# modichirag/GSM-VI

Hardware: AMD Instinct MI355X
Metric: GSM updates/sec at D=1024,B=32 (dense-cov gsm_update, fp64) (higher is better)
Workload: dtype f64; 1 GPU; BASELINE configs[2]: D=1024 dense-cov Gaussian target, B=32, one GSM update per step; D=1024, B=32, instances=21, ring_bytes=352321536, launch=hipGraph(90 x 21 updates/replay + 1 x 7), warmup_steps_run=28, parallelism=single GPU

## Files before the change

### gsm-vi_amd/csrc/gsmvi_abi.hip

```cpp
#include <hip/hip_runtime.h>

#include <cstdio>
#include <cstdlib>
#include <cstring>
#include <string>

#include "../../include/gsmvi_hip.h"
#include "../../include/gsmvi_hip_debug.h"

void gsmvi_launch_panel_partial(hipStream_t st, hipEvent_t* ev, int MT, dim3 grid, int D, int ncols, int nrows,
                                const double* A, int lda, const double* shift, double alpha, const double* M,
                                int ldm, double* Pp, int chunks_per_wg, int a_vec_ok);
void gsmvi_launch_panel_finish(hipStream_t st, hipEvent_t* ev, int D, int nrows, int KC, const double* Pp,
                               const double* addvec, double* Out, int ldo, int ncols_out);
void gsmvi_launch_gsm_scalars(hipStream_t st, hipEvent_t* ev, int D, int B, int KC, const double* X, int ldx,
                              const double* G, int ldg, const double* mu0, const double* Pp, double* rec,
                              int ldrec);
size_t gsmvi_cov_update_lds_bytes(int SB);
hipError_t gsmvi_cov_update_prepare();
hipError_t gsmvi_bam_prepare();
hipError_t gsmvi_batched_prepare();
hipError_t gsmvi_bam_batched_prepare();
hipError_t gsmvi_psis_batched_prepare();
hipError_t gsmvi_psis_loo_batched_prepare();
hipError_t gsmvi_psis_loo_softmax_batched_prepare();
hipError_t gsmvi_softmax_predict_batched_prepare();
void gsmvi_launch_gsm_cov_update(hipStream_t st, hipEvent_t* ev, int D, int B, const double* rec, int ldrec,
                                 const double* mu0, const double* S0, int lds0, double* S, int lds, double* mu_out,
                                 int SB, int s_vec_ok, int row0, int nrows);
int gsmvi_panel_t_product(struct gsmvi_ctx* ctx, hipStream_t st, int D, int B, const double* A, int lda,
                          const double* M, int ldm, int mrows, double* Pp, int* kc_out);
void gsmvi_launch_commit(hipStream_t st, int D, const int* info, const double* mu_new, const double* S_new,
                         int lds_new, double* mu, double* S, int lds, int* n_reverts);
void gsmvi_launch_panel_fast(hipStream_t st, hipEvent_t* ev, int MT, dim3 grid, int D, int nrows, const double* A,
                             int lda, const double* shift, double alpha, const double* M, int ldm, double* Pp,
                             int chunks_per_wg, int ncols, unsigned long long* stamps, double* Out, int ldo,
                             const double* addvec, const struct gsmvi_panel_extras* px);
bool gsmvi_launch_gsm_scalars_fast(hipStream_t st, hipEvent_t* ev, int D, int B, int KC, const double* X, int ldx,
                                   const double* G, int ldg, const double* mu0, const double* Pp, double* rec,
                                   int ldrec, int nt, unsigned long long* stamps);
bool gsmvi_launch_gsm_cov_sym(hipStream_t st, hipEvent_t* ev, int D, int B, const double* rec, int ldrec,
                              const double* mu0, const double* S0, int lds0, double* S, int lds, double* mu_out,
                              int dbg, unsigned long long* stamps, int num_cu);
void gsmvi_launch_panel_fast_part(hipStream_t st, hipEvent_t* ev, dim3 grid, int D, int B, const double* G, int ldg,
                                  const double* S0, int lds0, double* Pp, int chunks_per_wg, const double* X, int ldx,
                                  const double* mu0, double* Qg, double* Qm, int chw, bool qm_whole, int stream,
                                  unsigned long long* stamps);
void gsmvi_launch_gsm_cov_sym_slabs(hipStream_t st, hipEvent_t* ev, int D, int B, const struct gsm_slab_src& fs, const double* mu0,
                                    const double* S0, int lds0, double* S, int lds, double* mu_out, int kct, bool fold,
                                    bool s0_last, bool store_wt, bool qm_whole, unsigned long long* stamps);
int gsmvi_cov_sym_pairs(int nt);
int gsmvi_panel_fast_chunk(int MT);
int gsmvi_potrf_impl(struct gsmvi_ctx* ctx, hipStream_t st, int D, const double* S, int lds, double* R, int ldr,
                     int* info_dev);
int gsmvi_gram_impl(hipStream_t st, int D, const double* F, int ldf, double* C, int ldc, double shift, const double* shift_dev);
int gsmvi_whiten_impl(hipStream_t st, int D, int nrows, const double* R, int ldr, const double* X, int ldx,
                      const double* mu, double* Z, int ldz, double* logdiag);
int gsmvi_factor_impl(struct gsmvi_ctx* ctx, hipStream_t st, int D, int B, const double* Z, int ldz, const double* X,
                      int ldx, const double* G, int ldg, const double* mu0, const double* F0, int ldf0, double* mu,
                      double* F, int ldf, int* info_dev, int* n_reverts_dev);
int gsmvi_factor_local_impl(struct gsmvi_ctx* ctx, hipStream_t st, int D, int Bl, const double* Z, int ldz,
                            const double* X, int ldx, const double* G, int ldg, const double* mu0, const double* F0,
                            int ldf0, double* rec, int ldrec);
int gsmvi_factor_apply_impl(struct gsmvi_ctx* ctx, hipStream_t st, int D, int B, const double* Z, int ldz,
                            const double* rec, int ldrec, const double* mu0, const double* F0, int ldf0, double* mu,
                            double* F, int ldf, int* info_dev, int* n_reverts_dev);
int gsmvi_factor_apply_cols_impl(struct gsmvi_ctx* ctx, hipStream_t st, int D, int B, int col0, int ncols, const double* Z,
                                 int ldz, const double* W, int ldw, const double* X, int ldx, const double* mu0,
                                 const double* F0c, int ldf0, double* mu, double* Fc, int ldf, int* info_dev,
                                 int* n_reverts_dev);
int gsmvi_bam_impl(struct gsmvi_ctx* ctx, hipStream_t st, int D, int B, const double* X, int ldx,
                   const double* G, int ldg, const double* mu0, const double* S0, int lds0, double reg,
                   double jitter, double* mu, double* S, int lds, int* info_dev);
int gsmvi_bam_factor_impl(gsmvi_ctx* ctx, hipStream_t st, int D, int B, const double* Z, int ldz, const double* X, int ldx,
                          const double* G, int ldg, const double* mu0, const double* F0, int ldf0, double reg, double* mu,
                          double* F, int ldf, int* info_dev, int* n_reverts_dev);
int gsmvi_bam_factor_wq_partial_impl(gsmvi_ctx* ctx, hipStream_t st, int D, int B, int col0, int ncols, const double* G, int ldg,
                                     const double* F0c, int ldf0, double reg, double* Wq_part);
int gsmvi_bam_factor_apply_cols_impl(gsmvi_ctx* ctx, hipStream_t st, int D, int B, int col0, int ncols, const double* Z, int ldz,
                                     const double* X, int ldx, const double* G, int ldg, const double* Wq, const double* mu0,
                                     const double* F0c, int ldf0, double reg, double* mu, double* Fc, int ldf, int* info_dev,
                                     int* n_reverts_dev);

#include "gsmvi_ctx.h"
#include "gsmvi_panel_split.h"

static thread_local std::string g_last_error;

void gsmvi_set_error(const char* fmt, const char* a, const char* b) {
    char buf[512];
    snprintf(buf, sizeof buf, fmt, a ? a : "", b ? b : "");
    g_last_error = buf;
}

#define HIP_TRY(expr)                                                     \
    do {                                                                  \
        hipError_t e_ = (expr);                                           \
        if (e_ != hipSuccess) {                                           \
            gsmvi_set_error("%s failed: %s", #expr, hipGetErrorString(e_)); \
            return GSMVI_ERR_HIP;                                         \
        }                                                                 \
    } while (0)

// ... 156 lines not shown

int gsmvi_destroy(gsmvi_ctx* ctx) {
    if (!ctx) return GSMVI_OK;
    int prev_device = 0;
    (void)hipGetDevice(&prev_device);
    struct device_guard {
        int prev;
        ~device_guard() { (void)hipSetDevice(prev); }
    } guard{prev_device};
    (void)hipSetDevice(ctx->device);
    for (int k = 0; k < 8; ++k)
        if (ctx->ev[k]) (void)hipEventDestroy(ctx->ev[k]);
    if (ctx->ev_fork) (void)hipEventDestroy(ctx->ev_fork);
    if (ctx->ev_join) (void)hipEventDestroy(ctx->ev_join);
    if (ctx->side) (void)hipStreamDestroy(ctx->side);
    if (ctx->bam_hint_host) (void)hipHostFree(ctx->bam_hint_host);
    if (ctx->stamps) (void)hipFree(ctx->stamps);
    hipError_t e = hipFree(ctx->ws);
    delete ctx;
    if (e != hipSuccess) {
        gsmvi_set_error("hipFree failed: %s%s", hipGetErrorString(e), "");
        return GSMVI_ERR_HIP;
    }
    return GSMVI_OK;
}

int gsmvi_set_tuning(gsmvi_ctx* ctx, const char* name, int value) {
    BAD_ARG(!ctx || !name, "NULL argument");
    if (!strcmp(name, "panel_kc")) ctx->tune_panel_kc = value;
    else if (!strcmp(name, "update_sb")) ctx->tune_update_sb = value;
    else if (!strcmp(name, "no_fast")) ctx->tune_no_fast = value;
    else if (!strcmp(name, "direct_out")) ctx->tune_direct_out = value;
    else if (!strcmp(name, "rider")) ctx->tune_rider = value;
    else if (!strcmp(name, "potrf_split_m")) ctx->tune_potrf_split_m = value;
    else if (!strcmp(name, "potrf_dag")) ctx->tune_potrf_dag = value;
    else if (!strcmp(name, "panel_w4_min_D")) ctx->tune_panel_w4_min_D = value;
    else if (!strcmp(name, "potrf_spin")) ctx->tune_potrf_spin = value;
    else if (!strcmp(name, "potrf_workers")) ctx->tune_potrf_workers = value;
    else if (!strcmp(name, "wide")) ctx->tune_wide = value;
    else if (!strcmp(name, "wide_kc")) ctx->tune_wide_kc = value;
    else if (!strcmp(name, "fork_min_D")) ctx->tune_fork_min_D = value;
    else if (!strcmp(name, "gram_mt")) ctx->tune_gram_mt = value > 0 ? value : 4;
    else if (!strcmp(name, "bam_full")) ctx->tune_bam_full = value;
    else if (!strcmp(name, "bam_kenq")) ctx->tune_bam_kenq = value;
    else if (!strcmp(name, "bam_hint_slack")) ctx->tune_bam_hint_slack = value;
    else if (!strcmp(name, "rider_direct_max_D")) ctx->tune_rider_direct_max_D = value;
    else if (!strcmp(name, "chain_pair")) ctx->tune_chain_pair = value;
    else if (!strcmp(name, "bam_batched_pad")) ctx->tune_bam_batched_pad = value;
    else if (!strcmp(name, "lowrank_kp")) ctx->tune_lowrank_kp = value;
    else if (!strcmp(name, "bam_basis")) ctx->tune_bam_basis = value;
    else if (!strcmp(name, "scalars_nt")) ctx->tune_scalars_nt = value;
    else if (!strcmp(name, "gsm_two_launch")) ctx->tune_gsm_two_launch = value;
    else if (!strcmp(name, "cov_fold_diag")) ctx->tune_cov_fold_diag = value;
    else if (!strcmp(name, "cov_s0_last")) ctx->tune_cov_s0_last = value;
    else if (!strcmp(name, "cov_store_wt")) ctx->tune_cov_store_wt = value;
    else if (!strcmp(name, "panel_qm_whole")) ctx->tune_panel_qm_whole = value;
    else if (!strcmp(name, "panel_stream")) ctx->tune_panel_stream = value;
    else if (!strcmp(name, "cov_dbg")) ctx->tune_cov_dbg = value;
    else if (!strcmp(name, "timeline")) {
        if (value && !ctx->stamps) {
            HIP_TRY(hipMalloc(reinterpret_cast<void**>(&ctx->stamps), GSMVI_STAMP_WORDS * sizeof(unsigned long long)));
            HIP_TRY(hipMemset(ctx->stamps, 0, GSMVI_STAMP_WORDS * sizeof(unsigned long long)));
        }
        ctx->tune_timeline = value;
    }
    else {
        gsmvi_set_error("%s: unknown tuning knob %s", __func__, name);
        return GSMVI_ERR_BAD_ARG;
    }
    return GSMVI_OK;
}

int gsmvi_debug_stream_copy_f64(void* stream, double* dst, const double* src, size_t n) {
    BAD_ARG(!dst || !src || n < 2 || (n & 1) || (reinterpret_cast<uintptr_t>(dst) & 15u) || (reinterpret_cast<uintptr_t>(src) & 15u),
            "bad argument (16-byte aligned pointers, even n)");
    hipLaunchKernelGGL(k_stream_copy, dim3(2048), dim3(256), 0, static_cast<hipStream_t>(stream),
                       reinterpret_cast<const v2d_abi*>(src), reinterpret_cast<v2d_abi*>(dst), n / 2);
    return hipGetLastError() == hipSuccess ? GSMVI_OK : GSMVI_ERR_HIP;
}

int gsmvi_debug_read_stamps(gsmvi_ctx* ctx, unsigned long long* out, int n) {
    BAD_ARG(!ctx || !out || n < 1, "bad argument");
    HIP_TRY(hipDeviceSynchronize());
    if (ctx->tune_timeline && ctx->stamps) {
        BAD_ARG(n > GSMVI_STAMP_WORDS, "more words than the timeline buffer holds");
        HIP_TRY(hipMemcpy(out, ctx->stamps, sizeof(unsigned long long) * (size_t)n, hipMemcpyDeviceToHost));
        return GSMVI_OK;
    }
    HIP_TRY(hipMemcpy(out, ctx->pp, sizeof(unsigned long long) * (size_t)n, hipMemcpyDeviceToHost));
    return GSMVI_OK;
}

static double* ws_region(const gsmvi_ctx* ctx, int region) { return region == 0 ? ctx->pp : (region == 1 ? ctx->sg : ctx->small); }

int gsmvi_debug_read_workspace(gsmvi_ctx* ctx, int region, size_t offset, double* out, size_t n) {
    BAD_ARG(!ctx || !out || region < 0 || region > 2, "bad argument");
    const double* base = ws_region(ctx, region);
    HIP_TRY(hipDeviceSynchronize());
    HIP_TRY(hipMemcpy(out, base + offset, sizeof(double) * n, hipMemcpyDeviceToHost));
    return GSMVI_OK;
}

int gsmvi_debug_workspace_ptr(gsmvi_ctx* ctx, int region, double** out) {
    BAD_ARG(!ctx || !out || region < 0 || region > 2, "bad argument");
    *out = ws_region(ctx, region);
    return GSMVI_OK;
// ... 224 lines not shown
    return check_launch("k_gsm_scalars");
}

static bool gsm_two_launch_gate(const gsmvi_ctx* ctx, int D, int B, const double* X, int ldx, const double* G, int ldg,
                                const double* mu0, const double* S0, int lds0, const double* S, int lds, int* cpw_out,
                                int* kc_out, int* chw_out) {
    if (!ctx->tune_gsm_two_launch || ctx->tune_no_fast || ctx->tune_cov_dbg) return false;
    if (B != 16 && B != 32) return false;
    if (D % 256 != 0 || D > 1024) return false;
    if (ldx % 2 != 0 || ldg % 2 != 0 || lds0 % 2 != 0 || lds % 2 != 0) return false;
    if (!aligned16(X) || !aligned16(G) || !aligned16(mu0) || !aligned16(S0) || !aligned16(S)) return false;
    const int strips = D / 16, nchunks = D / 256;
    const gsmvi_panel_split sp = gsmvi_panel_split_k(strips, nchunks, ctx->tune_panel_kc, ctx->num_cu, GSMVI_MAX_KC);
    if (sp.kc > 4 || sp.kc * sp.cpw != nchunks) return false;
    *cpw_out = sp.cpw;
    *kc_out = sp.kc;
    *chw_out = 256;
    if (nchunks == 4 && ctx->tune_panel_kc <= 0) {
        *cpw_out = 1;
        *kc_out = 2;
        *chw_out = 512;
    }
    return true;
}

static int gsm_two_launch(gsmvi_ctx* ctx, hipStream_t hs, int D, int B, int cpw, int kc, int chw, const double* X, int ldx,
                          const double* G, int ldg, const double* mu0, const double* S0, int lds0, double* mu, double* S,
                          int lds) {
    const int strips = D / 16;
    double* Qg = ctx->sg;
    double* Qm = Qg + (size_t)B * kc * strips;
    ctx->px = gsmvi_panel_extras();
    ctx->px_used = 1;
    hipEvent_t* ev0 = ctx->stage_events(0);
    ctx->ev_valid[1] = 0;
    const bool qm_whole = chw == 512 && D == 1024 && ctx->tune_panel_qm_whole != 0;
    const int stream = (chw == 512 && D == 1024 && cpw == 1 && !qm_whole && ctx->tune_panel_stream != 0) ? (ctx->tune_panel_stream == 4 ? 4 : 2) : 0;
    gsmvi_launch_panel_fast_part(hs, ev0, dim3(strips, kc, chw == 512 ? B / 16 : 1), D, B, G, ldg, S0, lds0, ctx->pp, cpw, X, ldx, mu0, Qg, Qm, chw,
                                 qm_whole, stream, ctx->timeline_stamps(0));
    ctx->path |= GSMVI_PATH_PANEL_FAST | (chw == 512 ? GSMVI_PATH_PANEL_CHUNK512 : 0u) | (qm_whole ? GSMVI_PATH_PANEL_QM_WHOLE : 0u);
    int st = check_launch("k_panel_fast(partials)");
    if (st != GSMVI_OK) return st;
    gsm_slab_src fs;
    fs.X = X;
    fs.ldx = ldx;
    fs.Pp = ctx->pp;
    fs.Qg = Qg;
    fs.Qm = Qm;
    fs.KC = kc;
    fs.strips = strips;
    const bool fold = ctx->tune_cov_fold_diag >= 2 || (ctx->tune_cov_fold_diag == 1 && gsmvi_cov_sym_pairs(D / 32) >= ctx->num_cu);
    const bool s0_last = chw == 512 && ctx->tune_cov_s0_last != 0;
    const bool store_wt = chw == 512 && ctx->tune_cov_store_wt != 0 && (size_t)D * (size_t)lds * sizeof(double) < ((size_t)1 << 31);
    gsmvi_launch_gsm_cov_sym_slabs(hs, ctx->stage_events(2), D, B, fs, mu0, S0, lds0, S, lds, mu, chw == 512 ? 2 : 4, fold,
                                   s0_last, store_wt, qm_whole, ctx->timeline_stamps(2));
    ctx->path |= GSMVI_PATH_COV_SYM | GSMVI_PATH_GSM_TWO_LAUNCH | (fold ? GSMVI_PATH_COV_FOLD_DIAG : 0u) |
                 (s0_last ? GSMVI_PATH_COV_S0_LAST : 0u) | (store_wt ? GSMVI_PATH_COV_STORE_WT : 0u);
    return check_launch("k_gsm_cov_sym(slabs)");
}

int gsmvi_gsm_update_f64(gsmvi_ctx* ctx, void* stream, int D, int B, const double* X, int ldx, const double* G,
                         int ldg, const double* mu0, const double* S0, int lds0, double* mu, double* S, int lds) {
    int st = check_common(ctx, D, B, __func__);
    if (st != GSMVI_OK) return st;
    BAD_ARG(!X || !G || !mu0 || !S0 || !mu || !S, "NULL array");
    BAD_ARG(ldx < D || ldg < D || lds0 < D || lds < D, "leading dimension smaller than D");
    BAD_ARG(S == S0 || mu == mu0, "outputs must not alias inputs");
    hipStream_t hs = reinterpret_cast<hipStream_t>(stream);
    const int ldrec = 3 * D + (D & 1);
    int cpw2 = 0, kc2 = 0, chw2 = 0;
    if (gsm_two_launch_gate(ctx, D, B, X, ldx, G, ldg, mu0, S0, lds0, S, lds, &cpw2, &kc2, &chw2))
        return gsm_two_launch(ctx, hs, D, B, cpw2, kc2, chw2, X, ldx, G, ldg, mu0, S0, lds0, mu, S, lds);
    st = gsm_local_stage(ctx, hs, D, B, X, ldx, G, ldg, mu0, S0, lds0, ctx->sg, ldrec);
    if (st != GSMVI_OK) return st;
    return gsm_apply(ctx, hs, D, B, ctx->sg, ldrec, mu0, S0, lds0, mu, S, lds);
}

int gsmvi_gsm_record_len(int D) { return 3 * D + (D & 1); }

int gsmvi_gsm_update_general_f64(gsmvi_ctx* ctx, void* stream, int D, int B, const double* X, int ldx, const double* G,
                                 int ldg, const double* mu0, const double* S0, int lds0, double* mu, double* S, int lds) {
    int st = check_common(ctx, D, B, __func__);
    if (st != GSMVI_OK) return st;
    BAD_ARG(!X || !G || !mu0 || !S0 || !mu || !S, "NULL array");
    BAD_ARG(ldx < D || ldg < D || lds0 < D || lds < D, "leading dimension smaller than D");
    BAD_ARG(S == S0 || mu == mu0, "outputs must not alias inputs");
    hipStream_t hs = reinterpret_cast<hipStream_t>(stream);
    const int ldrec = 3 * D + (D & 1);
    int kc = 1;
    st = gsmvi_panel_t_product(ctx, hs, D, B, G, ldg, S0, lds0, D, ctx->pp, &kc);
    if (st != GSMVI_OK) return st;
    st = gsm_records(ctx, hs, D, B, kc, X, ldx, G, ldg, mu0, ctx->pp, ctx->sg, ldrec);
    if (st != GSMVI_OK) return st;
    const int SB = cov_update_sb(B, 0);
    const int s_vec_ok = (lds0 % 2 == 0) && (lds % 2 == 0) && aligned16(S0) && aligned16(S);
    ctx->path |= GSMVI_PATH_COV_GENERIC;
    gsmvi_launch_gsm_cov_update(hs, nullptr, D, B, ctx->sg, ldrec, mu0, S0, lds0, S, lds, mu, SB, s_vec_ok, 0, D);
    return check_launch("k_gsm_cov_update(general)");
}

int gsmvi_gsm_local_stage_f64(gsmvi_ctx* ctx, void* stream, int D, int B_local, const double* X, int ldx,
                              const double* G, int ldg, const double* mu0, const double* S0, int lds0, double* rec,
                              int ldrec) {
    int st = check_common(ctx, D, B_local, __func__);
    if (st != GSMVI_OK) return st;
    BAD_ARG(!X || !G || !mu0 || !S0 || !rec, "NULL array");
    BAD_ARG(ldx < D || ldg < D || lds0 < D || ldrec < 3 * D, "leading dimension too small");
    hipStream_t hs = reinterpret_cast<hipStream_t>(stream);
    return gsm_local_stage(ctx, hs, D, B_local, X, ldx, G, ldg, mu0, S0, lds0, rec, ldrec);
// ... 257 lines not shown
```

### gsm-vi_amd/csrc/gsmvi_ctx.h

```cpp
#pragma once
#include <hip/hip_runtime.h>
#include <cstddef>

#define GSMVI_MAX_KC 8
#define GSMVI_FACTOR_NMAX 256
#define GSMVI_STAMP_WORDS (4 * 4096)

struct gsmvi_panel_extras {
    const double* msl = nullptr;
    int kcm = 0;
    size_t mstride = 0;
    int ldsl = 0, msplit = 0;
    double* mfin = nullptr;
    int ldfin = 0;
    const double* sj_src = nullptr;
    int sj_kc = 0;
    size_t sj_stride = 0;
    int sj_len = 0;
    double* sj_dst = nullptr;
    int rd_on = 0, rd_n = 0, rd_B = 0, rd_kcg = 0, rd_jmode = 0;
    const double* rd_Gp = nullptr;
    double *rd_Kmat = nullptr, *rd_coef = nullptr;
    int* rd_bad = nullptr;
    unsigned long long* rd_stamps = nullptr;
// ... 14 lines not shown

struct bam_reg {
    double v;
    const double* p;
#if defined(__HIPCC__)
    __device__ __forceinline__ double get() const { return p ? *p : v; }
#endif
};

struct gsmf_bam_mean {
    const double* xbar;
    const double* sg_r1;
    bam_reg reg;
};

struct gsmvi_ctx {
    gsmvi_panel_extras px;
    int px_used = 0;
    unsigned path = 0;
    int tune_panel_w4_min_D = 2048;
    int colwin_0 = 0, colwin_n = 0;
    const double* potrf_w = nullptr;
    const double* potrf_r = nullptr;
    int potrf_w_n = 0;
    int tune_potrf_dag = 1;
    int tune_potrf_workers = 0;
    int tune_potrf_spin = 0;
    int tune_potrf_split_m = 0;
    int tune_wide = 1;
    int tune_wide_kc = 0;
    int tune_gram_mt = 1;
    int tune_rider = 1;
    int device = 0;
    int max_D = 0, max_B = 0;
    int num_cu = 256;
    int rmax = 0;
    void* ws = nullptr;
    size_t ws_bytes = 0;
    double* pp = nullptr;
    double* sg = nullptr;
    double *fo_Rt = nullptr, *fo_Tm = nullptr, *fo_Fs = nullptr;
    double* small = nullptr;
    int* ints = nullptr;
    double* gram_slabs = nullptr;
    int tune_panel_kc = 0;
    int tune_update_sb = 0;
    int tune_cov_dbg = 0;
    int tune_timeline = 0;
    unsigned long long* stamps = nullptr;
    int tune_direct_out = 1;
    int tune_scalars_nt = 0;
    int tune_no_fast = 0;
    int tune_cov_fold_diag = 1;
    int tune_cov_s0_last = 1;
    int tune_cov_store_wt = 1;
    int tune_panel_qm_whole = 0;
    int tune_panel_stream = 1;
    int tune_gsm_two_launch = 1;
    int* bam_hint_host = nullptr;
    int tune_bam_kenq = 0;
    int tune_bam_hint_slack = 1;
    int tune_rider_direct_max_D = 2048;
    int tune_bam_full = 0;
    int tune_lowrank_kp = 0;
    int tune_bam_batched_pad = 1;
    int tune_chain_pair = 1;
    gsmf_bam_mean bam_mean = {nullptr, nullptr, {0.0, nullptr}};
    int bam_mean_done = 0;
    const double* chain_r11 = nullptr;
    const double* chain_w11 = nullptr;
    const double* reg_dev = nullptr;
    int tune_bam_basis = 1;
    double* basis = nullptr;
    const double* chain_pi = nullptr;
    double* chain_x = nullptr;
    double* early = nullptr;
    int early_ready = 0;
    int profiling = 0;
    hipStream_t side = nullptr;
    hipEvent_t ev_fork = nullptr, ev_join = nullptr;
    int tune_fork_min_D = 3072;
    hipEvent_t ev[8] = {};
    int ev_valid[4] = {};

    unsigned long long* timeline_stamps(int kernel) {
        return (tune_timeline && stamps) ? stamps + (size_t)kernel * 4096 : nullptr;
    }

    hipEvent_t* stage_events(int stage) {
        if (!profiling) return nullptr;
        ev_valid[stage] = 1;
        return &ev[2 * stage];
    }
};

void gsmvi_panel_wide_split(int D, int tiles, int num_cu, int kc_force, int* kc_out, int* kper_out);
void gsmvi_launch_panel_wide(hipStream_t st, hipEvent_t* ev, bool transposed, int D, int nrows, const double* A, int lda,
                             const double* shift, double alpha, const double* M, int ldm, double* Pp, int kper, int kc,
                             int ncols);
int gsmvi_panel_product_nc(gsmvi_ctx* ctx, hipStream_t st, hipEvent_t* ev, int D, int ncols, int nrows,
                           const double* A, int lda, const double* shift, double alpha, const double* M, int ldm,
                           double* Pp, int* kc_out);
int gsmvi_panel_product_out(gsmvi_ctx* ctx, hipStream_t st, int D, int ncols, int nrows, const double* A, int lda,
                            const double* shift, double alpha, const double* M, int ldm, const double* addvec, double* Out,
                            int ldo);
int gsmvi_panel_finish(hipStream_t st, int ncols, int nrows, int kc, const double* Pp, const double* addvec,
// ... 16 lines not shown
```

### gsm-vi_amd/csrc/gsmvi_fast.hip

```cpp
#include "gsmvi_common.h"
#include "gsmvi_ctx.h"
#include "gsmvi_small16.h"
#include <hip/hip_ext.h>

#define GSMVI_LAUNCH(kern, grid, block, shmem, st, ev, ...)                                         \
    do {                                                                                           \
        if (ev)                                                                                    \
            hipExtLaunchKernelGGL(kern, grid, block, shmem, st, (ev)[0], (ev)[1], 0, __VA_ARGS__); \
        else                                                                                       \
            hipLaunchKernelGGL(kern, grid, block, shmem, st, __VA_ARGS__);                         \
    } while (0)

template <int NS>
__device__ __forceinline__ void panel_stream_chunk(double* As, int D, int nrows, const double* __restrict__ A, int lda, double alpha,
                                                   const double* __restrict__ M, int ldm, const gsmvi_panel_extras& px,
                                                   unsigned long long* __restrict__ stamps, v4d& acc, double& pq_g, double& pq_x,
                                                   double& pq_m) {
    static_assert(NS == 2 || NS == 4, "stages of the streamed left operand");
    constexpr int LDG = 514;
    constexpr int UPR = 32 / NS;
    constexpr int RPI = 64 / UPR;
    constexpr int IPS = 16 / RPI;
    constexpr int SPS = 16 / NS;
    const int tid = threadIdx.x, w = tid >> 6, l = tid & 63, c = l & 15, ks = l >> 4;
// ... 420 lines not shown
        gv[e] = G[(size_t)b * ldg + ic];
        mv0[e] = mu0[ic];
    }
    double p0 = 0.0, p1 = 0.0, sg[EPT], dd[EPT];
#pragma unroll
    for (int e = 0; e < EPT; ++e) {
        const int i = tid + NT * e;
        double t = 0.0;
#pragma unroll
        for (int kc = 0; kc < KCT; ++kc) t += (kc < KC) ? pp[e][kc] : 0.0;
        sg[e] = t;
        dd[e] = mv0[e] - xv[e];
        if (i < D) {
            p0 += gv[e] * t;
            p1 += dd[e] * gv[e];
        }
    }
    if (stamps && threadIdx.x == 0) stamps[(size_t)blockIdx.x * 8 + 1] = __builtin_amdgcn_s_memrealtime();
    p0 = wave_sum(p0);
    p1 = wave_sum(p1);
    const int w = tid >> 6;
    if ((tid & 63) == 0) {
        lds[2 * w] = p0;
        lds[2 * w + 1] = p1;
    }
    __syncthreads();
    double gSg = 0.0, mv = 0.0;
#pragma unroll
    for (int k = 0; k < NW; ++k) {
        gSg += lds[2 * k];
        mv += lds[2 * k + 1];
    }
    const double rho = 0.5 * sqrt(1.0 + 4.0 * (gSg + mv * mv)) - 0.5;
    const double den = 1.0 + rho + mv;
    const double beta = 1.0 / (1.0 + rho), c = (gSg - mv) / den;
    double* rb = rec + (size_t)b * ldrec;
#pragma unroll
    for (int e = 0; e < EPT; ++e) {
        const int i = tid + NT * e;
        if (i < D) {
            const double dmu = beta * ((sg[e] - dd[e]) - c * dd[e]);
            rb[i] = dd[e];
            rb[D + i] = dd[e] + dmu;
            rb[2 * D + i] = dmu;
        }
    }
    if (stamps) {
        asm volatile("s_waitcnt vmcnt(0)" ::: "memory");
        if (threadIdx.x == 0) stamps[(size_t)blockIdx.x * 8 + 3] = __builtin_amdgcn_s_memrealtime();
    }
}

typedef unsigned int v4u __attribute__((ext_vector_type(4)));
template <int SB, bool RAG, bool FROM_SLABS = false, int KCT = 4, bool FOLD = false, bool S0L = false, bool WT = false, bool QMW = false>
__global__ __launch_bounds__(512) __attribute__((amdgpu_waves_per_eu(FROM_SLABS ? 4 : 2))) void k_gsm_cov_sym(int D, int B, double invB, const double* __restrict__ rec, int ldrec,
                                                     const double* __restrict__ mu0,
                                                     const double* __restrict__ S0, int lds0,
                                                     double* __restrict__ S, int lds,
                                                     double* __restrict__ mu_out, int dbg,
                                                     unsigned long long* __restrict__ stamps, gsm_slab_src fs) {
    static_assert(!FOLD || FROM_SLABS, "folded diagonal tiles: the two-launch form only");
    static_assert(!(S0L || WT || QMW) || (FROM_SLABS && KCT == 2 && !RAG), "S0 last / write-through stores / whole-sample Qm: the two-slab two-launch form only, on the grid");
#define PRE_W_BARRIER()                                                                   \
    do {                                                                                  \
        if constexpr (S0L) asm volatile("s_waitcnt lgkmcnt(0)\n\ts_barrier" ::: "memory"); \
        else __syncthreads();                                                             \
    } while (0)
#define STAMP(k)                                                                          \
    do {                                                                                  \
        if (stamps && threadIdx.x == 0) stamps[(size_t)blockIdx.x * 8 + (k)] = __builtin_amdgcn_s_memrealtime(); \
    } while (0)
    if (blockIdx.x >= GSMVI_STAMP_WG) stamps = nullptr;
    STAMP(0);
    constexpr int RS = 48;
    constexpr int NPASS = (SB > 32) ? SB / 32 : 1;
    constexpr int SBP = SB / NPASS;
    constexpr int TILE = SBP * RS;
    constexpr int NU = SB * 16;
    constexpr int UPT = (6 * NU) / 512;
    static_assert((6 * NU) % 512 == 0, "tile units must divide over 512 threads");
    __shared__ __attribute__((aligned(16))) double smem[6 * TILE >= 2 * 32 * 33 ? 6 * TILE : 2 * 32 * 33];

    const int nt = (D + 31) >> 5;
    const int n_two = ((nt >> 1) * ((nt + 1) >> 1));
    int ti, tj0;
    bool two;
    int fold = 0;
    if (FOLD || (int)blockIdx.x < n_two) {
        int rem = blockIdx.x;
        ti = 0;
        for (;;) {
            const int inrow = (nt - ti) >> 1;
            if (rem < inrow) break;
            rem -= inrow;
            ++ti;
        }
        tj0 = ti + ((nt - ti) & 1) + 2 * rem;
        two = true;
        if constexpr (FOLD) fold = (((nt - ti) & 1) && rem == 0) ? 1 : (ti == nt - 2 ? 2 : 0);
    } else {
        const int k = blockIdx.x - n_two;
        ti = ((nt & 1) ? 0 : 1) + 2 * k;
        tj0 = ti;
        two = false;
    }
    const bool diag = (tj0 == ti);
    const int I0 = ti * 32, J0 = tj0 * 32;
    const int tid = threadIdx.x, w = tid >> 6, l = tid & 63, c = l & 15, ks = l >> 4;
    const int t = w >> 2;
    const int wr = (w >> 1) & 1, wc = w & 1;
    const bool mine = (t == 0) || two;

    const int Jt = J0 + 32 * ((t == 1 && two) ? 1 : 0);
    const int tl = tid & 255;
    v2d s0v[2];
    if constexpr (!S0L) {
#pragma unroll
        for (int q = 0; q < 2; ++q) {
            const int unit = q * 256 + tl, i = unit >> 4, j2 = unit & 15;
            const int gr = (RAG && I0 + i >= D) ? D - 1 : I0 + i, gc = (RAG && Jt + 2 * j2 >= D) ? D - 2 : Jt + 2 * j2;
            s0v[q] = (dbg & 2) ? (v2d){1.0, 1.0} : *reinterpret_cast<const v2d*>(S0 + (size_t)gr * lds0 + gc);
        }
    }
    const int X0 = (fold == 2) ? J0 + 32 : I0;
    v2d s0x = {0.0, 0.0};
    if constexpr (FOLD && !S0L) {
        if (fold) s0x = *reinterpret_cast<const v2d*>(S0 + (size_t)(X0 + (tid >> 4)) * lds0 + X0 + 2 * (tid & 15));
    }
    if constexpr (!S0L) __builtin_amdgcn_sched_barrier(0);
    v2d stg[UPT];
    double dmu_part = 0.0;
    v2d dmuI = {0.0, 0.0};
    v2d dmuX = {0.0, 0.0};
    [[maybe_unused]] double mu0I = 0.0, mu0X = 0.0;
    if constexpr (FROM_SLABS) {
        static_assert(!RAG && NPASS == 1 && 512 % NU == 0, "two-launch form: B == SB in {16, 32}, on the grid");
        static_assert(KCT == 2 || KCT == 4, "slab count of the two-launch form");
        constexpr int NQG = 2 * KCT;
        const int u = tid & (NU - 1), b = u >> 4, ln = u & 15, c2 = 2 * ln;
        const bool st_d = (NU == 512) || tid < NU, st_e = (NU == 512) || tid >= NU;
        const int nqg = (fs.KC * fs.strips) >> 1, nqm = fs.strips >> 1;
// ... 681 lines not shown
    gsmvi_panel_extras px;
    px.sj_src = X;
    px.sj_len = ldx;
    px.msl = mu0;
    px.sj_dst = Qg;
    px.mfin = Qm;
#define PFQ(MTV, CW) GSMVI_LAUNCH((k_panel_fast<MTV, false, CW, false, false, false, true>), grid, dim3(512), 0, st, ev, D, B, G, ldg, \
                                  nullptr, 1.0, S0, lds0, Pp, chunks_per_wg, D, stamps, nullptr, 0, nullptr, px)
    if (chw == 512 && qm_whole)
        GSMVI_LAUNCH((k_panel_fast<1, false, 512, false, false, false, true, true>), grid, dim3(512), 0, st, ev, D, B, G, ldg, nullptr, 1.0, S0,
                     lds0, Pp, chunks_per_wg, D, stamps, nullptr, 0, nullptr, px);
    else if (chw == 512 && stream != 0 && chunks_per_wg == 1 && D == 512 * (int)grid.y && B % 16 == 0) {
#define PFS(NS) GSMVI_LAUNCH((k_panel_fast<1, false, 512, false, false, false, true, false, NS>), grid, dim3(512), 0, st, ev, D, B, G, ldg, \
                             nullptr, 1.0, S0, lds0, Pp, chunks_per_wg, D, stamps, nullptr, 0, nullptr, px)
        if (stream == 4) PFS(4); else PFS(2);
    } else if (chw == 512 && stamps != nullptr && chunks_per_wg == 1) {
        PFS(-1);
#undef PFS
    } else if (chw == 512) PFQ(1, 512);
    else { if (B == 16) PFQ(1, 256); else PFQ(2, 256); }
#undef PFQ
}

int gsmvi_panel_fast_chunk(int MT) { return MT == 4 ? 128 : 256; }

bool gsmvi_launch_gsm_scalars_fast(hipStream_t st, hipEvent_t* ev, int D, int B, int KC, const double* X, int ldx,
                                   const double* G, int ldg, const double* mu0, const double* Pp, double* rec,
                                   int ldrec, int nt, unsigned long long* stamps) {
    if (nt != 256 && nt != 512 && nt != 1024) nt = 512;
    const int ept = (D + nt - 1) / nt;
#define SF(E, K, N)                                                                                              \
    GSMVI_LAUNCH((k_gsm_scalars_fast<E, K, N>), dim3(B), dim3(N), 0, st, ev, D, B, KC, X, ldx, G, ldg, mu0, Pp, rec, \
                 ldrec, stamps)
#define SFK(E, N) do { if (kct == 1) SF(E, 1, N); else if (kct == 2) SF(E, 2, N); else if (kct == 4) SF(E, 4, N); else SF(E, 8, N); } while (0)
#define SFE(N) do { if (e == 1) SFK(1, N); else if (e == 2) SFK(2, N); else if (e == 4) SFK(4, N); else SFK(8, N); } while (0)
    if (KC > 8 || ept > 8) return false;
    const int kct = KC <= 1 ? 1 : (KC <= 2 ? 2 : (KC <= 4 ? 4 : 8));
    const int e = ept <= 1 ? 1 : (ept <= 2 ? 2 : (ept <= 4 ? 4 : 8));
    if (nt == 256) SFE(256); else if (nt == 512) SFE(512); else SFE(1024);
#undef SFE
#undef SFK
#undef SF
    return true;
}

static int cov_sym_grid(int nt) {
    int n = 0;
    for (int ti = 0; ti < nt; ++ti) n += (nt - ti + 1) / 2;
    return n;
}

int gsmvi_cov_sym_pairs(int nt) { return (nt >> 1) * ((nt + 1) >> 1); }

bool gsmvi_launch_gsm_cov_sym(hipStream_t st, hipEvent_t* ev, int D, int B, const double* rec, int ldrec,
                              const double* mu0, const double* S0, int lds0, double* S, int lds, double* mu_out,
                              int dbg, unsigned long long* stamps, int num_cu) {
    if (B < 1) return false;
    if (B > 128) {
        GSMVI_LAUNCH(k_gsm_cov_sym_big, dim3(cov_sym_grid((D + 31) / 32)), dim3(512), 0, st, ev, D, B, 1.0 / (double)B, rec, ldrec,
                     mu0, S0, lds0, S, lds, mu_out);
        return true;
    }
    const int SB = B <= 16 ? 16 : (B <= 32 ? 32 : (B <= 64 ? 64 : 128));
    const double invB = 1.0 / (double)B;
    const bool rag = D % 32 != 0 || B != SB;
    const int n_items = cov_sym_grid((D + 31) / 32);
    if (n_items >= 2048 && SB <= 32 && !stamps && dbg == 0) {
        const dim3 pgrid(2 * (num_cu > 0 ? num_cu : 256));
#define CSP(SBV, RG) GSMVI_LAUNCH((k_gsm_cov_sym_p<SBV, RG>), pgrid, dim3(512), 0, st, ev, D, B, invB, rec, ldrec, mu0, S0, lds0, S, lds, mu_out)
        if (rag) { if (SB == 16) CSP(16, true); else CSP(32, true); }
        else { if (SB == 16) CSP(16, false); else CSP(32, false); }
        return true;
#undef CSP
    }
    if (dbg & 512) dbg &= ~512;
    const dim3 grid(n_items);
#define CS(SBV, RG)                                                                                         \
    GSMVI_LAUNCH((k_gsm_cov_sym<SBV, RG>), grid, dim3(512), 0, st, ev, D, B, invB, rec, ldrec, mu0, S0, lds0, S, lds, mu_out, dbg, \
                 stamps, gsm_slab_src())
    if (rag) {
        switch (SB) {
            case 16: CS(16, true); break;
            case 32: CS(32, true); break;
            case 64: CS(64, true); break;
            default: CS(128, true); break;
        }
    } else {
        switch (SB) {
            case 16: CS(16, false); break;
            case 32: CS(32, false); break;
            case 64: CS(64, false); break;
            default: CS(128, false); break;
        }
    }
#undef CS
    return true;
}

void gsmvi_launch_gsm_cov_sym_slabs(hipStream_t st, hipEvent_t* ev, int D, int B, const gsm_slab_src& fs, const double* mu0,
                                    const double* S0, int lds0, double* S, int lds, double* mu_out, int kct, bool fold,
                                    bool s0_last, bool store_wt, bool qm_whole, unsigned long long* stamps) {
    const dim3 grid(fold ? gsmvi_cov_sym_pairs(D / 32) : cov_sym_grid(D / 32));
    const double invB = 1.0 / (double)B;
#define CSQ(SBV, KV, FV, LV, WV, QV)                                                                                      \
    GSMVI_LAUNCH((k_gsm_cov_sym<SBV, false, true, KV, FV, LV, WV, QV>), grid, dim3(512), 0, st, ev, D, B, invB, nullptr, 0, mu0, S0, lds0, S, \
                 lds, mu_out, 0, stamps, fs)
#define CSS(SBV, KV, FV, LV, WV) do { if (KV == 2 && qm_whole) CSQ(SBV, 2, FV, LV, WV, true); else CSQ(SBV, KV, FV, LV, WV, false); } while (0)
#define CSF(SBV, KV, LV, WV) do { if (fold) CSS(SBV, KV, true, LV, WV); else CSS(SBV, KV, false, LV, WV); } while (0)
#define CSL(SBV)                                                                                                          \
    do {                                                                                                                  \
        if (s0_last && store_wt) CSF(SBV, 2, true, true);                                                                 \
        else if (s0_last) CSF(SBV, 2, true, false);                                                                       \
        else if (store_wt) CSF(SBV, 2, false, true);                                                                      \
        else CSF(SBV, 2, false, false);                                                                                   \
    } while (0)
    if (kct == 2) { if (B == 16) CSL(16); else CSL(32); }
    else { if (B == 16) CSF(16, 4, false, false); else CSF(32, 4, false, false); }
#undef CSL
#undef CSF
#undef CSS
#undef CSQ
}
```

Before: 70110 updates/s.

## Handle diagonal tile pairs as 64x64 quads in the slab covariance kernel

Adds a 'quad' variant of the two-launch symmetric covariance update. Each of the first nt/2 workgroups handles a 64x64 diagonal block made of two diagonal 32x32 tiles plus their off-diagonal tile, computed with MFMA from staged d/e tiles, and also produces the mu_out update. The remaining workgroups take the strictly off-diagonal pairs, giving a grid of (nt/2)^2 instead of the fold layout. It is enabled by default when the fold path would be selected at chw=512 with S0-last and write-through stores. The aim is to balance per-workgroup work and avoid the folded diagonal handling, at the cost of a larger LDS footprint and a much more complex diagonal code path.

New measurement: 71810 updates/s, median of 6. 1.02x the previous value.

```diff
diff --git a/gsm-vi_amd/csrc/gsmvi_abi.hip b/gsm-vi_amd/csrc/gsmvi_abi.hip
--- a/gsm-vi_amd/csrc/gsmvi_abi.hip
+++ b/gsm-vi_amd/csrc/gsmvi_abi.hip
@@ -48,7 +48,7 @@
                                   unsigned long long* stamps);
 void gsmvi_launch_gsm_cov_sym_slabs(hipStream_t st, hipEvent_t* ev, int D, int B, const struct gsm_slab_src& fs, const double* mu0,
                                     const double* S0, int lds0, double* S, int lds, double* mu_out, int kct, bool fold,
-                                    bool s0_last, bool store_wt, bool qm_whole, unsigned long long* stamps);
+                                    bool s0_last, bool store_wt, bool qm_whole, bool quad, unsigned long long* stamps);
 int gsmvi_cov_sym_pairs(int nt);
 int gsmvi_panel_fast_chunk(int MT);
 int gsmvi_potrf_impl(struct gsmvi_ctx* ctx, hipStream_t st, int D, const double* S, int lds, double* R, int ldr,
@@ -311,6 +311,7 @@
     else if (!strcmp(name, "scalars_nt")) ctx->tune_scalars_nt = value;
     else if (!strcmp(name, "gsm_two_launch")) ctx->tune_gsm_two_launch = value;
     else if (!strcmp(name, "cov_fold_diag")) ctx->tune_cov_fold_diag = value;
+    else if (!strcmp(name, "cov_diag_quad")) ctx->tune_cov_diag_quad = value;
     else if (!strcmp(name, "cov_s0_last")) ctx->tune_cov_s0_last = value;
     else if (!strcmp(name, "cov_store_wt")) ctx->tune_cov_store_wt = value;
     else if (!strcmp(name, "panel_qm_whole")) ctx->tune_panel_qm_whole = value;
@@ -641,9 +642,12 @@
     const bool fold = ctx->tune_cov_fold_diag >= 2 || (ctx->tune_cov_fold_diag == 1 && gsmvi_cov_sym_pairs(D / 32) >= ctx->num_cu);
     const bool s0_last = chw == 512 && ctx->tune_cov_s0_last != 0;
     const bool store_wt = chw == 512 && ctx->tune_cov_store_wt != 0 && (size_t)D * (size_t)lds * sizeof(double) < ((size_t)1 << 31);
+    const bool quad_form = chw == 512 ? (s0_last && store_wt && !qm_whole) : true;
+    const bool quad = quad_form && ((ctx->tune_cov_diag_quad >= 2 && ctx->tune_cov_fold_diag != 0) ||
+                                    (ctx->tune_cov_diag_quad == 1 && chw == 512 && ctx->tune_cov_fold_diag == 1 && fold));
     gsmvi_launch_gsm_cov_sym_slabs(hs, ctx->stage_events(2), D, B, fs, mu0, S0, lds0, S, lds, mu, chw == 512 ? 2 : 4, fold,
-                                   s0_last, store_wt, qm_whole, ctx->timeline_stamps(2));
-    ctx->path |= GSMVI_PATH_COV_SYM | GSMVI_PATH_GSM_TWO_LAUNCH | (fold ? GSMVI_PATH_COV_FOLD_DIAG : 0u) |
+                                   s0_last, store_wt, qm_whole, quad, ctx->timeline_stamps(2));
+    ctx->path |= GSMVI_PATH_COV_SYM | GSMVI_PATH_GSM_TWO_LAUNCH | ((fold || quad) ? GSMVI_PATH_COV_FOLD_DIAG : 0u) |
                  (s0_last ? GSMVI_PATH_COV_S0_LAST : 0u) | (store_wt ? GSMVI_PATH_COV_STORE_WT : 0u);
     return check_launch("k_gsm_cov_sym(slabs)");
 }
diff --git a/gsm-vi_amd/csrc/gsmvi_ctx.h b/gsm-vi_amd/csrc/gsmvi_ctx.h
--- a/gsm-vi_amd/csrc/gsmvi_ctx.h
+++ b/gsm-vi_amd/csrc/gsmvi_ctx.h
@@ -90,6 +90,7 @@
     int tune_scalars_nt = 0;
     int tune_no_fast = 0;
     int tune_cov_fold_diag = 1;
+    int tune_cov_diag_quad = 1;
     int tune_cov_s0_last = 1;
     int tune_cov_store_wt = 1;
     int tune_panel_qm_whole = 0;
diff --git a/gsm-vi_amd/csrc/gsmvi_fast.hip b/gsm-vi_amd/csrc/gsmvi_fast.hip
--- a/gsm-vi_amd/csrc/gsmvi_fast.hip
+++ b/gsm-vi_amd/csrc/gsmvi_fast.hip
@@ -496,7 +496,255 @@
 }
 
 typedef unsigned int v4u __attribute__((ext_vector_type(4)));
-template <int SB, bool RAG, bool FROM_SLABS = false, int KCT = 4, bool FOLD = false, bool S0L = false, bool WT = false, bool QMW = false>
+template <int SB>
+constexpr int COV_QUAD_SCR = (3 * 32 * 33 + 2 * SB * 32 + 512 > 4 * SB * 48) ? 3 * 32 * 33 + 2 * SB * 32 + 512 : 4 * SB * 48;
+template <int SB>
+constexpr int COV_QUAD_LDS = COV_QUAD_SCR<SB> + 512;
+
+template <int SB, int KCT, bool S0L, bool WT>
+__device__ __forceinline__ void gsm_cov_quad(double* __restrict__ smem, int p, int D, int B, double invB, const double* __restrict__ mu0,
+                                             const double* __restrict__ S0, int lds0, double* __restrict__ S, int lds,
+                                             double* __restrict__ mu_out, unsigned long long* __restrict__ stamps, const gsm_slab_src& fs) {
+#define QBARRIER()                                                                        \
+    do {                                                                                  \
+        if constexpr (S0L) asm volatile("s_waitcnt lgkmcnt(0)\n\ts_barrier" ::: "memory"); \
+        else __syncthreads();                                                             \
+    } while (0)
+#define QSTAMP(k)                                                                         \
+    do {                                                                                  \
+        if (stamps && threadIdx.x == 0) stamps[(size_t)blockIdx.x * 8 + (k)] = __builtin_amdgcn_s_memrealtime(); \
+    } while (0)
+    constexpr int RS = 48, TILE = SB * RS, NU = SB * 16, NS = SB / 4, NQG = 2 * KCT;
+    constexpr int LWS = 32 * 33, MUO = 3 * LWS, PAO = MUO + 2 * SB * 32, SCO = COV_QUAD_SCR<SB>;
+    static_assert(512 % NU == 0 && (KCT == 2 || KCT == 4), "two-launch form: B == SB in {16, 32}");
+    static_assert(SCO >= 4 * TILE && SCO >= PAO + 512, "handed-over accumulators outside the staged tiles and the store path's LDS");
+    const int A0 = 64 * p, B0 = A0 + 32;
+    const int tid = threadIdx.x, w = tid >> 6, l = tid & 63, c = l & 15, ks = l >> 4;
+    const int t = w >> 2, wr = (w >> 1) & 1, wc = w & 1, tl = tid & 255;
+    const int Jt = t ? B0 : A0;
+    const int u = tid & (NU - 1), b = u >> 4, ln = u & 15, c2 = 2 * ln;
+    const bool st_d = (NU == 512) || tid < NU, st_e = (NU == 512) || tid >= NU;
+    const int nqg = (fs.KC * fs.strips) >> 1, nqm = fs.strips >> 1;
+    auto ld16 = [](const double* base, unsigned byte_off) {
+        return *reinterpret_cast<const v2d*>(reinterpret_cast<const char*>(base) + byte_off);
+    };
+    v2d s0v[2], s0x;
+    auto load_s0 = [&]() {
+#pragma unroll
+        for (int q = 0; q < 2; ++q) {
+            const int unit = q * 256 + tl;
+            s0v[q] = *reinterpret_cast<const v2d*>(S0 + (size_t)(A0 + (unit >> 4)) * lds0 + Jt + 2 * (unit & 15));
+        }
+        s0x = *reinterpret_cast<const v2d*>(S0 + (size_t)(B0 + (tid >> 4)) * lds0 + B0 + 2 * (tid & 15));
+    };
+    if constexpr (!S0L) {
+        load_s0();
+        __builtin_amdgcn_sched_barrier(0);
+    }
+    const unsigned qg0 = (unsigned)(b * nqg) * 16u, qm0 = (unsigned)(b * nqm) * 16u;
+    v2d qg[NQG], qm[2];
+#pragma unroll
+    for (int k = 0; k < NQG; ++k) qg[k] = ld16(fs.Qg, qg0 + 16u * (unsigned)(ln + 16 * k < nqg ? ln + 16 * k : nqg - 1));
+#pragma unroll
+    for (int k = 0; k < 2; ++k) qm[k] = ld16(fs.Qm, qm0 + 16u * (unsigned)(ln + 16 * k < nqm ? ln + 16 * k : nqm - 1));
+    double mu0q = 0.0;
+    if (w == 0) mu0q = mu0[A0 + l];
+    const int col[2] = {A0 + c2, B0 + c2};
+    const size_t slab = (size_t)B * D;
+    v2d xv[2], m0[2], sl[2][KCT];
+    auto load_block = [&](int cb) {
+        xv[cb] = *reinterpret_cast<const v2d*>(fs.X + (size_t)b * fs.ldx + col[cb]);
+        m0[cb] = ld16(mu0, 8u * (unsigned)col[cb]);
+#pragma unroll
+        for (int kc = 0; kc < KCT; ++kc)
+            sl[cb][kc] = *reinterpret_cast<const v2d*>(fs.Pp + (size_t)(KCT == 2 ? kc : (kc < fs.KC ? kc : fs.KC - 1)) * slab + (size_t)b * D + col[cb]);
+    };
+    load_block(0);
+    if constexpr (KCT == 2) load_block(1);
+    if constexpr (S0L) {
+        __builtin_amdgcn_sched_barrier(0);
+        load_s0();
+        __builtin_amdgcn_sched_barrier(0);
+    }
+    double gs = 0.0, ms = 0.0;
+#pragma unroll
+    for (int k = 0; k < NQG; ++k) {
+        const bool in = ln + 16 * k < nqg;
+        gs += in ? qg[k].x : 0.0;
+        gs += in ? qg[k].y : 0.0;
+    }
+#pragma unroll
+    for (int k = 0; k < 2; ++k) {
+        const bool in = ln + 16 * k < nqm;
+        ms += in ? qm[k].x : 0.0;
+        ms += in ? qm[k].y : 0.0;
+    }
+    if constexpr (KCT == 4) {
+        asm volatile("" : "+v"(gs), "+v"(ms) : : "memory");
+        load_block(1);
+    }
+    const double gSg = row16_sum(gs);
+    const double mv = row16_sum(ms);
+    const double rho = 0.5 * sqrt(1.0 + 4.0 * (gSg + mv * mv)) - 0.5;
+    const double den = 1.0 + rho + mv;
+    double beta = 1.0 / (1.0 + rho), cc = (gSg - mv) / den;
+    if (stamps) {
+        if constexpr (S0L) asm volatile("s_waitcnt vmcnt(3)" ::: "memory");
+        else asm volatile("s_waitcnt vmcnt(0)" ::: "memory");
+        QSTAMP(1);
+    }
+    v2d dmuq[2];
+#pragma unroll
+    for (int cb = 0; cb < 2; ++cb) {
+        v2d sg = {0.0, 0.0}, dd, dm, ee;
+        if constexpr (KCT == 2) {
+            if (cb == 0) asm volatile("" : "+v"(beta), "+v"(cc), "+v"(xv[0]), "+v"(m0[0]), "+v"(sl[0][0]), "+v"(sl[0][1]));
+            else asm volatile("" : "+v"(xv[cb]), "+v"(m0[cb]), "+v"(sl[cb][0]), "+v"(sl[cb][1]));
+            sg.x = sl[cb][0].x + sl[cb][1].x;
+            sg.y = sl[cb][0].y + sl[cb][1].y;
+        } else {
+#pragma unroll
+            for (int kc = 0; kc < 4; ++kc) {
+                sg.x += (kc < fs.KC) ? sl[cb][kc].x : 0.0;
+                sg.y += (kc < fs.KC) ? sl[cb][kc].y : 0.0;
+            }
+        }
+        dd.x = m0[cb].x - xv[cb].x;
+        dd.y = m0[cb].y - xv[cb].y;
+        dm.x = beta * ((sg.x - dd.x) - cc * dd.x);
+        dm.y = beta * ((sg.y - dd.y) - cc * dd.y);
+        ee.x = dd.x + dm.x;
+        ee.y = dd.y + dm.y;
+        if (st_d) *reinterpret_cast<v2d*>(smem + (2 * cb) * TILE + b * RS + c2) = dd;
+        if (st_e) *reinterpret_cast<v2d*>(smem + (2 * cb + 1) * TILE + b * RS + c2) = ee;
+        dmuq[cb] = dm;
+    }
+    QBARRIER();
+    QSTAMP(2);
+    v4d accd = {0.0, 0.0, 0.0, 0.0}, acce = {0.0, 0.0, 0.0, 0.0}, xacc = {0.0, 0.0, 0.0, 0.0};
+    {
+        const int ta = (w == 3) ? 2 : 0, tb = (w >= 3) ? 2 : 0;
+        const int br = (w >= 4) ? wr : (w == 2 ? 1 : 0), bc = (w >= 4) ? wc : ((w == 1 || w == 2) ? 1 : 0);
+        const double* adp = smem + ta * TILE + ks * RS + 16 * br + c;
+        const double* bdp = smem + tb * TILE + ks * RS + 16 * bc + c;
+        double ad[NS], ae[NS], bd[NS], be[NS];
+#pragma unroll
+        for (int s = 0; s < NS; ++s) {
+            ad[s] = adp[4 * s * RS];
+            ae[s] = adp[TILE + 4 * s * RS];
+            bd[s] = bdp[4 * s * RS];
+            be[s] = bdp[TILE + 4 * s * RS];
+        }
+#pragma unroll
+        for (int s = 0; s < NS; ++s) {
+            accd = GSMVI_MFMA_F64(ad[s], bd[s], accd);
+            acce = GSMVI_MFMA_F64(ae[s], be[s], acce);
+        }
+        if (w < 4) {
+            const double* xp = smem + (2 + (w & 1)) * TILE + ks * RS + c;
+#pragma unroll
+            for (int s = 0; s < NS; ++s) {
+                ad[s] = xp[4 * s * RS + 16 * (w >> 1)];
+                bd[s] = xp[4 * s * RS + 16];
+            }
+#pragma unroll
+            for (int s = 0; s < NS; ++s) xacc = GSMVI_MFMA_F64(ad[s], bd[s], xacc);
+            if (!(w & 1)) {
+#pragma unroll
+                for (int r = 0; r < 4; ++r) smem[SCO + (w >> 1) * 256 + r * 64 + l] = xacc[r];
+            }
+        }
+    }
+    QBARRIER();
+    {
+        const int lw = (w >= 4) ? 1 : (w == 3 ? 2 : 0);
+        const int br = (w >= 4) ? wr : (w == 2 ? 1 : 0), bc = (w >= 4) ? wc : ((w == 1 || w == 2) ? 1 : 0);
+        double* LW = smem + lw * LWS;
+#pragma unroll
+        for (int r = 0; r < 4; ++r) {
+            const double v = (accd[r] - acce[r]) * invB;
+            LW[(16 * br + ks + 4 * r) * 33 + 16 * bc + c] = v;
+            if (w == 1) LW[(16 + c) * 33 + ks + 4 * r] = v;
+        }
+        if (w < 4 && (w & 1)) {
+            double* LX = smem + 2 * LWS;
+#pragma unroll
+            for (int r = 0; r < 4; ++r) {
+                const double v = (smem[SCO + (w >> 1) * 256 + r * 64 + l] - xacc[r]) * invB;
+                LX[(16 * (w >> 1) + ks + 4 * r) * 33 + 16 + c] = v;
+                if (w == 1) LX[(16 + c) * 33 + ks + 4 * r] = v;
+            }
+        }
+    }
+    if (tid < NU) {
+        *reinterpret_cast<v2d*>(smem + MUO + (tid >> 4) * 32 + 2 * (tid & 15)) = dmuq[0];
+        *reinterpret_cast<v2d*>(smem + MUO + SB * 32 + (tid >> 4) * 32 + 2 * (tid & 15)) = dmuq[1];
+    }
+    QSTAMP(3);
+    QBARRIER();
+    if constexpr (S0L) {
+        if (stamps) { asm volatile("s_waitcnt vmcnt(0)" ::: "memory"); QSTAMP(6); }
+    }
+    [[maybe_unused]] __amdgpu_buffer_rsrc_t srs;
+    if constexpr (WT) srs = __builtin_amdgcn_make_buffer_rsrc(S, 0, (int)(((size_t)(D - 1) * lds + D) * sizeof(double)), 0x00020000);
+    auto store_s = [&](size_t off, v2d v) {
+        if constexpr (WT) __builtin_amdgcn_raw_buffer_store_b128(__builtin_bit_cast(v4u, v), srs, (int)(off * sizeof(double)), 0, 16);
+        else *reinterpret_cast<v2d*>(S + off) = v;
+    };
+    {
+        const double* mt = smem + MUO + (tid >> 8) * SB * 32;
+        double part = 0.0;
+#pragma unroll
+        for (int k = 0; k < SB / 8; ++k) part += mt[(((tid >> 5) & 7) + 8 * k) * 32 + (tid & 31)];
+        smem[PAO + tid] = part;
+    }
+    {
+        double* LW = smem + t * LWS;
+#pragma unroll
+        for (int q = 0; q < 2; ++q) {
+            const int unit = q * 256 + tl, i = unit >> 4, j2 = unit & 15;
+            v2d wv2;
+            wv2.x = s0v[q].x + LW[i * 33 + 2 * j2];
+            wv2.y = s0v[q].y + LW[i * 33 + 2 * j2 + 1];
+            store_s((size_t)(A0 + i) * lds + Jt + 2 * j2, wv2);
+            if (t) {
+                LW[i * 33 + 2 * j2] = wv2.x;
+                LW[i * 33 + 2 * j2 + 1] = wv2.y;
+            }
+        }
+    }
+    {
+        const int i = tid >> 4, j2 = tid & 15;
+        v2d wv2;
+        wv2.x = s0x.x + smem[2 * LWS + i * 33 + 2 * j2];
+        wv2.y = s0x.y + smem[2 * LWS + i * 33 + 2 * j2 + 1];
+        store_s((size_t)(B0 + i) * lds + B0 + 2 * j2, wv2);
+    }
+    asm volatile("s_waitcnt lgkmcnt(0)\n\ts_barrier" ::: "memory");
+    if (t) {
+        const double* LW = smem + LWS;
+#pragma unroll
+        for (int q = 0; q < 2; ++q) {
+            const int unit = q * 256 + tl, j = unit >> 4, i2 = unit & 15;
+            v2d m2;
+            m2.x = LW[(2 * i2) * 33 + j];
+            m2.y = LW[(2 * i2 + 1) * 33 + j];
+            store_s((size_t)(B0 + j) * lds + A0 + 2 * i2, m2);
+        }
+    }
+    if (w == 0) {
+        double s = 0.0;
+#pragma unroll
+        for (int q = 0; q < 8; ++q) s += smem[PAO + (l >> 5) * 256 + q * 32 + (l & 31)];
+        mu_out[A0 + l] = mu0q + s * invB;
+    }
+    QSTAMP(4);
+    if (stamps) { asm volatile("s_waitcnt vmcnt(0)" ::: "memory"); QSTAMP(5); }
+#undef QSTAMP
+#undef QBARRIER
+}
+
+template <int SB, bool RAG, bool FROM_SLABS = false, int KCT = 4, bool FOLD = false, bool S0L = false, bool WT = false, bool QMW = false, bool QUAD = false>
 __global__ __launch_bounds__(512) __attribute__((amdgpu_waves_per_eu(FROM_SLABS ? 4 : 2))) void k_gsm_cov_sym(int D, int B, double invB, const double* __restrict__ rec, int ldrec,
                                                      const double* __restrict__ mu0,
                                                      const double* __restrict__ S0, int lds0,
@@ -505,6 +753,7 @@
                                                      unsigned long long* __restrict__ stamps, gsm_slab_src fs) {
     static_assert(!FOLD || FROM_SLABS, "folded diagonal tiles: the two-launch form only");
     static_assert(!(S0L || WT || QMW) || (FROM_SLABS && KCT == 2 && !RAG), "S0 last / write-through stores / whole-sample Qm: the two-slab two-launch form only, on the grid");
+    static_assert(!QUAD || (FROM_SLABS && !FOLD && !QMW && !RAG && (SB == 16 || SB == 32)), "quads: the two-launch form, in place of the fold");
 #define PRE_W_BARRIER()                                                                   \
     do {                                                                                  \
         if constexpr (S0L) asm volatile("s_waitcnt lgkmcnt(0)\n\ts_barrier" ::: "memory"); \
@@ -523,14 +772,30 @@
     constexpr int NU = SB * 16;
     constexpr int UPT = (6 * NU) / 512;
     static_assert((6 * NU) % 512 == 0, "tile units must divide over 512 threads");
-    __shared__ __attribute__((aligned(16))) double smem[6 * TILE >= 2 * 32 * 33 ? 6 * TILE : 2 * 32 * 33];
+    constexpr int QLDS = QUAD ? COV_QUAD_LDS<SB> : 0;
+    __shared__ __attribute__((aligned(16))) double smem[6 * TILE >= 2 * 32 * 33 ? (6 * TILE >= QLDS ? 6 * TILE : QLDS) : 2 * 32 * 33];
 
     const int nt = (D + 31) >> 5;
     const int n_two = ((nt >> 1) * ((nt + 1) >> 1));
     int ti, tj0;
     bool two;
     int fold = 0;
-    if (FOLD || (int)blockIdx.x < n_two) {
+    if constexpr (QUAD) {
+        if ((int)blockIdx.x < (nt >> 1)) {
+            gsm_cov_quad<SB, KCT, S0L, WT>(smem, blockIdx.x, D, B, invB, mu0, S0, lds0, S, lds, mu_out, stamps, fs);
+            return;
+        }
+        int rem = blockIdx.x - (nt >> 1);
+        ti = 0;
+        for (;;) {
+            const int inrow = (nt >> 1) - (ti >> 1) - 1;
+            if (rem < inrow) break;
+            rem -= inrow;
+            ++ti;
+        }
+        tj0 = 2 * ((ti >> 1) + 1) + 2 * rem;
+        two = true;
+    } else if (FOLD || (int)blockIdx.x < n_two) {
         int rem = blockIdx.x;
         ti = 0;
         for (;;) {
@@ -1318,6 +1583,8 @@
 
 int gsmvi_cov_sym_pairs(int nt) { return (nt >> 1) * ((nt + 1) >> 1); }
 
+static int cov_sym_quad_grid(int nt) { return (nt >> 1) * (nt >> 1); }
+
 bool gsmvi_launch_gsm_cov_sym(hipStream_t st, hipEvent_t* ev, int D, int B, const double* rec, int ldrec,
                               const double* mu0, const double* S0, int lds0, double* S, int lds, double* mu_out,
                               int dbg, unsigned long long* stamps, int num_cu) {
@@ -1365,9 +1632,19 @@
 
 void gsmvi_launch_gsm_cov_sym_slabs(hipStream_t st, hipEvent_t* ev, int D, int B, const gsm_slab_src& fs, const double* mu0,
                                     const double* S0, int lds0, double* S, int lds, double* mu_out, int kct, bool fold,
-                                    bool s0_last, bool store_wt, bool qm_whole, unsigned long long* stamps) {
+                                    bool s0_last, bool store_wt, bool qm_whole, bool quad, unsigned long long* stamps) {
+    const double invB = 1.0 / (double)B;
+    if (quad) {
+        const dim3 qgrid(cov_sym_quad_grid(D / 32));
+#define CSD(SBV, KV, LV, WV)                                                                                              \
+    GSMVI_LAUNCH((k_gsm_cov_sym<SBV, false, true, KV, false, LV, WV, false, true>), qgrid, dim3(512), 0, st, ev, D, B, invB, nullptr, 0, mu0, \
+                 S0, lds0, S, lds, mu_out, 0, stamps, fs)
+        if (kct == 2) { if (B == 16) CSD(16, 2, true, true); else CSD(32, 2, true, true); }
+        else { if (B == 16) CSD(16, 4, false, false); else CSD(32, 4, false, false); }
+#undef CSD
+        return;
+    }
     const dim3 grid(fold ? gsmvi_cov_sym_pairs(D / 32) : cov_sym_grid(D / 32));
-    const double invB = 1.0 / (double)B;
 #define CSQ(SBV, KV, FV, LV, WV, QV)                                                                                      \
     GSMVI_LAUNCH((k_gsm_cov_sym<SBV, false, true, KV, FV, LV, WV, QV>), grid, dim3(512), 0, st, ev, D, B, invB, nullptr, 0, mu0, S0, lds0, S, \
                  lds, mu_out, 0, stamps, fs)
```
